# stephane-caron/qpmpc

Hardware: AMD Instinct MI355X
Metric: MPC QP builds+solves/sec (batched) (higher is better)
Workload: dtype f64

## Files before the change

qpmpc_amd/csrc/mpcqp_quad.hip:

```cpp
#include <hip/hip_runtime.h>
#include <math.h>
#include <stdint.h>
#include <type_traits>

#include "mpcqp.h"
#include "mpcqp_internal.h"
#include "mpcqp_quad_common.h"

namespace mpcqp {

namespace quad {

constexpr int MMAX = 32;
constexpr int MK = 2;

}

using namespace quad;

template <int NX, bool ORD, int WPB, bool SLIM, bool MODEL = false, bool GEN = false>
__global__ void __launch_bounds__(64 * WPB, SLIM ? 2 : 1)
    mpcqp_quad_kernel(const double *__restrict__ gA, const double *__restrict__ gB, const double *__restrict__ gC,
                      const double *__restrict__ ge, const double *__restrict__ gx0, const double *__restrict__ ggoal,
                      const double *__restrict__ gtgt, double *__restrict__ oU, double *__restrict__ olam, int32_t *__restrict__ ostatus,
                      int32_t *__restrict__ oiters, const KernelArgs ka, const int64_t batch)
{
    using T = double;
    extern __shared__ __attribute__((aligned(16))) unsigned char smem_raw[];
    {
        const int64_t b0 = ka.A.batch_stride, b1 = ka.B.batch_stride, b2 = ka.C.batch_stride, b3 = ka.e.batch_stride,
                      b4 = ka.x0.batch_stride, b5 = ka.goal.batch_stride;
        const int64_t s0 = ka.A.step_stride, s1 = ka.B.step_stride, s2 = ka.C.step_stride, s3 = ka.e.step_stride;
        asm volatile("" ::"s"(b0), "s"(b1), "s"(b2), "s"(b3), "s"(b4), "s"(b5), "s"(s0), "s"(s1), "s"(s2), "s"(s3), "s"(ka.N), "s"(ka.nu),
                     "s"(ka.flags), "s"(ka.probe), "s"(gA), "s"(gB), "s"(gC), "s"(ge), "s"(gx0), "s"(ggoal), "s"(ka.n), "s"(ka.m),
                     "s"(batch));
    }
    const int lane = threadIdx.x & 63;
    const int wv = threadIdx.x >> 6;
    const int rb = lane & 48;
    const int l = lane & 15;
    int64_t prob = 4 * ((int64_t)blockIdx.x * WPB + wv) + (rb >> 4);
    const bool valid = prob < batch;
    prob = valid ? prob : batch - 1;
    if constexpr (ORD) {
        const int64_t o = ka.order[prob];
        prob = o < 0 ? 0 : (o >= batch ? batch - 1 : o);
    }
    using CV = Carve<SLIM>;
    constexpr int LDM = CV::LDM, PER = CV::PER;
    T *sm = (T *)smem_raw + (4 * wv + (rb >> 4)) * PER;
    const int n = ka.n, m = ka.m;
    const int row0 = l, row1 = l + NV;
    const bool isc0 = row0 < m, isc1 = row1 < m;
    const T INF = HUGE_VAL;
    constexpr int GS = 33;
    T *Gimg = sm + CV::OFF_M, *Ml = sm + CV::OFF_M;
    T *LTp = sm + CV::OFF_LT + (l * (31 - l)) / 2 - (l + 1);
    T *LTimg = sm + CV::OFF_LT, *Timg = sm + CV::OFF_T;
    int *actv = reinterpret_cast<int *>(sm + CV::OFF_ACT);

    long long *stamp = ka.probe ? (long long *)ka.probe + prob * 16 : nullptr;
    auto tick = [&](int slot) {
        if (stamp && l == 0 && valid) {
            stamp[slot] = (long long)__builtin_readcyclecounter();
            if (slot == 0 || slot == 6) stamp[slot ? 13 : 12] = (long long)__builtin_amdgcn_s_memrealtime();
        }
    };
    tick(0);

    T hval0, hval1;
    bool notpd = false;
    T RM0[NV], RM1[NV], RLt[NV];
    T wv_ = T(0);
    if constexpr (MODEL) {
        const T *model = gA;
        const ModelLayout ml = make_model_layout(ka.nx, ka.N, n, m);
        const int nxr = ka.nx, nT = ka.N * ka.nx;
        const T *x0 = gx0 + prob * ka.x0.batch_stride;
        const T *goal = ggoal ? ggoal + prob * ka.goal.batch_stride : nullptr;
        const T *tgt = gtgt ? gtgt + prob * ka.targets.batch_stride : nullptr;
        notpd = model[ml.total] != T(0);
        {
            T r0[NV], r1[NV];
            ld16(r0, model + ml.off_M + (size_t)(isc0 ? row0 : 0) * NV);
            ld16(r1, model + ml.off_M + (size_t)(isc1 ? row1 : 0) * NV);
            ld16(RLt, model + ml.off_LinvT + (size_t)l * NV);
#pragma unroll
            for (int k = 0; k < NV; ++k) {
                RM0[k] = isc0 ? r0[k] : T(0);
                RM1[k] = isc1 ? r1[k] : T(0);
            }
        }
        auto bound = [&](int row, bool isc) {
            if (!isc) return INF;
            const int mkr = ka.mk, kq = mkr == 2 ? row >> 1 : row / mkr;
            T hh = ge ? ge[prob * ka.e.batch_stride + kq * ka.e.step_stride + (row - kq * mkr)] : model[ml.off_e + row];
            for (int c = 0; c < nxr; ++c) hh -= model[ml.off_Hx + (size_t)row * nxr + c] * x0[c];
            return hh;
        };
        hval0 = bound(row0, isc0);
        hval1 = bound(row1, isc1);
        for (int c = 0; c < nxr; ++c) wv_ += model[ml.off_Wx + (size_t)l * nxr + c] * x0[c];
        if ((ka.flags & MPCQP_Q_TERMINAL) && goal)
            for (int c = 0; c < nxr; ++c) wv_ -= model[ml.off_Wg + (size_t)l * nxr + c] * goal[c];
        if ((ka.flags & MPCQP_Q_STAGE) && tgt)
            for (int j2 = 0; j2 < nT; ++j2) wv_ -= model[ml.off_Wt + (size_t)l * nT + j2] * tgt[j2];
        tick(1);
    } else {
    T Pr[NV];
    T qa;
    T g15a = T(0), g15b = T(0);
    {
        constexpr bool WIDE = GEN && NX > 6;
        const int nx = WIDE ? ka.nx : NX;
        const int nu = ka.nu, N = ka.N;
        constexpr int MKG = GEN ? 4 : MK;
        const int mk = GEN ? ka.mk : MK;
        auto stepof = [&](int row) { return mk == 2 ? row >> 1 : (mk == 1 ? row : (mk == 4 ? row >> 2 : row / 3)); };
        const T *A = gA + prob * ka.A.batch_stride;
        const T *B = gB + prob * ka.B.batch_stride;
        const bool hasC = !GEN || gC != nullptr;
        const T *Cm = hasC ? gC + prob * ka.C.batch_stride : A;
        const T *x0 = gx0 + prob * ka.x0.batch_stride;
        const T *goal = ggoal ? ggoal + prob * ka.goal.batch_stride : nullptr;
        const int sA = ka.A.step_stride ? nx * nx : 0, sB = ka.B.step_stride ? nx * nu : 0, sC = (hasC && ka.C.step_stride) ? mk * nx : 0;
        const bool termP = ka.flags & MPCQP_P_TERMINAL, termQ = (ka.flags & MPCQP_Q_TERMINAL) && goal;
        const T *Dm = (GEN && ka.D.ptr) ? (const T *)ka.D.ptr + prob * ka.D.batch_stride : nullptr;
        const T *tgt = (GEN && gtgt) ? gtgt + prob * ka.targets.batch_stride : nullptr;
        const int sD = (GEN && ka.D.step_stride) ? mk * nu : 0;
        const bool stageP = GEN && (ka.flags & MPCQP_P_STAGE), stageQ = GEN && (ka.flags & MPCQP_Q_STAGE) && tgt;
        constexpr int NAe = NX * NX, NEe = NAe + MKG * NX;
        const int NEr = hasC ? NAe + mk * NX : NAe;
        const bool col = (l < n);
        const int j = col ? (nu == 1 ? l : l / nu) : -1, ii = col ? l - j * nu : 0;
        const int64_t eb = prob * ka.e.batch_stride;
        const int kq0 = stepof(row0), kq1 = stepof(row1);
        const T eval0 = isc0 ? ge[eb + kq0 * ka.e.step_stride + (row0 - kq0 * mk)] : INF;
        const T eval1 = isc1 ? ge[eb + kq1 * ka.e.step_stride + (row1 - kq1 * mk)] : INF;
        const bool xl15 = (l == NV - 1);
        T v[NX], gref[NX], bcol[NX];
#pragma unroll
        for (int s = 0; s < NX; ++s) {
            v[s] = (xl15 && s < nx) ? x0[s < nx ? s : 0] : T(0);
            gref[s] = (termQ && s < nx) ? goal[s < nx ? s : 0] : T(0);
        }
#pragma unroll
        for (int r = 0; r < NX; ++r) bcol[r] = (col && r < nx) ? B[j * sB + (r < nx ? r : 0) * nu + ii] : T(0);
        T dcol[MKG], d15a = T(0), d15b = T(0), tg[NX];
#pragma unroll
        for (int u = 0; u < NX; ++u) tg[u] = T(0);
#pragma unroll
        for (int i2 = 0; i2 < MKG; ++i2) dcol[i2] = T(0);
        if constexpr (GEN) {
            if (Dm) {
#pragma unroll
                for (int i2 = 0; i2 < MKG; ++i2) dcol[i2] = (col && !xl15 && i2 < mk) ? Dm[j * sD + i2 * nu + ii] : T(0);
                if (n == NV) {
                    const int j15 = nu == 1 ? NV - 1 : (NV - 1) / nu, i15 = NV - 1 - j15 * nu;
                    d15a = (isc0 && kq0 == j15) ? Dm[j15 * sD + (row0 - kq0 * mk) * nu + i15] : T(0);
                    d15b = (isc1 && kq1 == j15) ? Dm[j15 * sD + (row1 - kq1 * mk) * nu + i15] : T(0);
                }
            }
            if (stageQ && !WIDE) {
#pragma unroll
                for (int u = 0; u < NX; ++u) tg[u] = (l + 16 * u < N * NX) ? tgt[l + 16 * u] : T(0);
            }
        }
        if constexpr (!WIDE) {
        constexpr int NOP = (NEe + 15) / 16;
        T op[NOP][NV];
        static_for<0, NOP>([&](auto rc) {
            constexpr int r = decltype(rc)::value;
            const int e = l + 16 * r;
            const bool ok = e < NEr;
            const T *p = (e < NAe) ? A + e : Cm + (ok ? e - NAe : 0);
            const int st = (e < NAe) ? sA : sC;
#pragma unroll
            for (int k = 0; k < NV; ++k) {
                const int kc = (k < N) ? k : N - 1;
                op[r][k] = p[kc * st];
            }
        });
        tick(8);
        const T wu = (T)ka.wu;
        qa = T(0);
#pragma unroll
        for (int b = 0; b < NV; ++b) Pr[b] = (l == b) ? (col ? wu : T(1)) : T(0);
        tick(9);
        auto mac = [&](auto idx, auto kc_, T &acc, T xx) {
            constexpr int IDX = decltype(idx)::value, K = decltype(kc_)::value;
            fmac_bcast<IDX % 16>(acc, op[IDX / 16][K], xx);
        };
        static_for<0, NV>([&](auto kk) {
            constexpr int k = decltype(kk)::value;
            if (k < N) {
                if constexpr (!GEN) {
                    T g[MK];
                    static_for<0, MK>([&](auto i2c) {
                        constexpr int i2 = decltype(i2c)::value;
                        T acc = T(0);
                        static_for<0, NX>([&](auto sc) {
                            constexpr int s2 = decltype(sc)::value;
                            mac(ic<NAe + i2 * NX + s2>{}, kk, acc, v[s2]);
                        });
                        g[i2] = acc;
                    });
#pragma unroll
                    for (int i2 = 0; i2 < MK; ++i2) Gimg[l * GS + k * MK + i2] = g[i2];
                } else {
                    static_for<0, MKG>([&](auto i2c) {
                        constexpr int i2 = decltype(i2c)::value;
                        if (i2 < mk) {
                            T acc = T(0);
                            if (hasC) {
                                static_for<0, NX>([&](auto sc) {
                                    constexpr int s2 = decltype(sc)::value;
                                    mac(ic<NAe + i2 * NX + s2>{}, kk, acc, v[s2]);
                                });
                            }
                            acc += (j == k) ? dcol[i2] : T(0);
                            Gimg[l * GS + k * mk + i2] = acc;
                        }
                    });
                }
                if constexpr (GEN && k >= 1) {
                    if (stageP || stageQ) {
                        const T wxs = (T)ka.wx;
                        static_for<0, NX>([&](auto sc) {
                            constexpr int s2 = decltype(sc)::value;
                            constexpr int te = k * NX + s2;
                            T src = xl15 ? T(0) : v[s2];
                            const T t = wxs * src;
                            if (stageQ) qa += t * (row_bcast<NV - 1>(v[s2]) - row_bcast<te % 16>(tg[te / 16]));
                            if (stageP) {
                                dpp_ready(src);
                                static_for<0, NV>([&](auto bc) { fmac_bcast<decltype(bc)::value>(Pr[decltype(bc)::value], src, t); });
                            }
                        });
                    }
                }
                const T hk = (j == k && !xl15) ? T(1) : T(0);
                T w[NX];
                static_for<0, NX>([&](auto rc) {
                    constexpr int r = decltype(rc)::value;
                    T acc = hk * bcol[r];
                    static_for<0, NX>([&](auto sc) {
                        constexpr int s2 = decltype(sc)::value;
                        mac(ic<r * NX + s2>{}, kk, acc, v[s2]);
                    });
                    w[r] = acc;
                });
#pragma unroll
                for (int r = 0; r < NX; ++r) v[r] = w[r];
            }
        });
        } else {
        tick(8);
        const T wu = (T)ka.wu;
        qa = T(0);
#pragma unroll
        for (int b = 0; b < NV; ++b) Pr[b] = (l == b) ? (col ? wu : T(1)) : T(0);
        tick(9);
        constexpr int NAw = NX * NX, NCw = 4 * NX, NEw = NAw + NCw + NX, NOPW = (NEw + 15) / 16;
        T opw[2][NOPW];
        auto fetch = [&](auto dc, int k) {
            constexpr int d = decltype(dc)::value;
            const int kc = k < N ? k : N - 1;
            static_for<0, NOPW>([&](auto rc) {
                constexpr int r = decltype(rc)::value;
                constexpr int e0 = 16 * r;
                const int e = e0 + l;
                T val;
                if constexpr (e0 < NAw) {
                    const int rr = e / NX, ss = e - rr * NX;
                    const bool ok = rr < nx && ss < nx;
                    val = A[kc * sA + (ok ? rr * nx + ss : 0)];
                    val = ok ? val : T(0);
                } else if constexpr (e0 < NAw + NCw) {
                    const int e2 = e - NAw, i2 = e2 / NX, ss = e2 - i2 * NX;
                    const bool ok = hasC && i2 < mk && ss < nx;
                    val = Cm[ok ? kc * sC + i2 * nx + ss : 0];
                    val = ok ? val : T(0);
                } else {
                    const int ss = e - NAw - NCw;
                    const bool ok = stageQ && ss < nx;
                    val = ok ? tgt[kc * nx + ss] : T(0);
                }
                opw[d][r] = val;
            });
        };
        fetch(ic<0>{}, 0);
        fetch(ic<1>{}, 1);
        const T wxs = (T)ka.wx;
        auto cstep = [&](auto dc, int k) {
            constexpr int d = decltype(dc)::value;
            static_for<0, NOPW>([&](auto rc) { dpp_ready(opw[d][decltype(rc)::value]); });
            static_for<0, 4>([&](auto i2c) {
                constexpr int i2 = decltype(i2c)::value;
                if (i2 < mk) {
                    T acc = T(0);
                    if (hasC) {
                        static_for<0, NX>([&](auto sc) {
                            constexpr int s2 = decltype(sc)::value, E = NAw + i2 * NX + s2;
                            fmac_bcast<E % 16>(acc, opw[d][E / 16], v[s2]);
                        });
                    }
                    acc += (j == k) ? dcol[i2] : T(0);
                    Gimg[l * GS + k * mk + i2] = acc;
                }
            });
            if (k >= 1 && (stageP || stageQ)) {
                static_for<0, NX>([&](auto sc) {
                    constexpr int s2 = decltype(sc)::value, E = NAw + NCw + s2;
                    T src = xl15 ? T(0) : v[s2];
                    const T t = wxs * src;
                    if (stageQ) qa += t * (row_bcast<NV - 1>(v[s2]) - row_bcast<E % 16>(opw[d][E / 16]));
                    if (stageP) {
                        dpp_ready(src);
                        static_for<0, NV>([&](auto bc) { fmac_bcast<decltype(bc)::value>(Pr[decltype(bc)::value], src, t); });
                    }
                });
            }
            const T hk = (j == k && !xl15) ? T(1) : T(0);
            T w[NX];
            static_for<0, NX>([&](auto rc) {
                constexpr int r = decltype(rc)::value;
                T acc = hk * bcol[r];
                static_for<0, NX>([&](auto sc) {
                    constexpr int s2 = decltype(sc)::value, E = r * NX + s2;
                    fmac_bcast<E % 16>(acc, opw[d][E / 16], v[s2]);
                });
                w[r] = acc;
            });
#pragma unroll
            for (int r = 0; r < NX; ++r) v[r] = w[r];
            fetch(dc, k + 2);
        };
        for (int k = 0; k < N; k += 2) {
            cstep(ic<0>{}, k);
            if (k + 1 < N) cstep(ic<1>{}, k + 1);
        }
        }
        tick(10);
        const T wt = (T)ka.wt;
        T x[NX];
#pragma unroll
        for (int s = 0; s < NX; ++s) {
            x[s] = row_bcast<NV - 1>(v[s]);
            v[s] = xl15 ? bcol[s] : v[s];
        }
#pragma unroll
        for (int s = 0; s < NX; ++s) {
            const T t = wt * v[s];
            if (termQ) qa += t * (x[s] - gref[s]);
            if (termP) {
                T src = v[s];
                dpp_ready(src);
                static_for<0, NV>([&](auto bc) { fmac_bcast<decltype(bc)::value>(Pr[decltype(bc)::value], src, t); });
            }
        }
        qa = col ? qa : T(0);
        tick(11);
        wave_sync();
        hval0 = isc0 ? eval0 - Gimg[(NV - 1) * GS + row0] : INF;
        hval1 = isc1 ? eval1 - Gimg[(NV - 1) * GS + row1] : INF;
        if constexpr (GEN) {
            g15a = d15a;
            g15b = d15b;
        }
    }
    tick(1);
    {
#pragma unroll
        for (int k = 0; k < NV; ++k) {
            RM0[k] = (isc0 && k < NV - 1) ? Gimg[k * GS + row0] : (GEN && k == NV - 1 ? g15a : T(0));
            RM1[k] = (isc1 && k < NV - 1) ? Gimg[k * GS + row1] : (GEN && k == NV - 1 ? g15b : T(0));
            RLt[k] = (l == k) ? T(1) : T(0);
        }
        static_for<0, NV>([&](auto jc) {
            constexpr int j = decltype(jc)::value;
            const T pij = Pr[j];
            const T piv = row_bcast<j>(pij);
            if (!(piv > T(0))) notpd = true;
            const T rinv = fast_rsqrt(piv);
            const T nt2 = -(pij * rinv * rinv);
            T nl = -(pij * rinv);
            RM0[j] *= rinv;
            RM1[j] *= rinv;
            RLt[j] *= rinv;
            const T wj = qa * rinv;
            wv_ = (l == j) ? wj : wv_;
            {
                T src = pij, wsrc = wj;
                asm volatile("s_nop 1" : "+v"(src), "+v"(nl), "+v"(wsrc) : "v"(RM0[j]), "v"(RM1[j]), "v"(RLt[j]));
                fmac_bcast<j>(qa, wsrc, nl);
                static_for<j + 1, NV>([&](auto kc) {
                    constexpr int k = decltype(kc)::value;
                    fmac_bcast<k>(Pr[k], src, nt2);
                    fmac_bcast<k>(RM0[k], nl, RM0[j]);
                    fmac_bcast<k>(RM1[k], nl, RM1[j]);
                    fmac_bcast<k>(RLt[k], nl, RLt[j]);
                });
            }
        });
        wave_sync();
    }
    }
    tick(2);
    tick(3);
    int status = MPCQP_MAX_ITER, iters = 0;
    T xsol = T(0);
    bool done = notpd;
    bool finished = notpd;
    if (notpd) status = MPCQP_NOT_PD;

    if (isc0) st16(Ml + row0 * LDM, RM0);
    if (isc1) st16(Ml + row1 * LDM, RM1);
    T ltd = T(0);
    if constexpr (SLIM) {
        static_for<0, NV>([&](auto kc) {
            constexpr int k = decltype(kc)::value;
            ltd = (l == k) ? RLt[k] : ltd;
            if (k > l) LTp[k] = RLt[k];
        });
    } else {
        st16(LTimg + l * NV, RLt);
    }
    const T y0 = -wv_;
    T s0, s1, invn0, invn1;
    {
        const T d0 = dot_bcast(wv_, RM0, hval0), d1 = dot_bcast(wv_, RM1, hval1);
        s0 = isc0 ? d0 : INF;
        s1 = isc1 ? d1 : INF;
        const T nn0 = dot16(RM0, RM0), nn1 = dot16(RM1, RM1);
        invn0 = (nn0 > T(0)) ? fast_rsqrt(nn0) : T(1);
        invn1 = (nn1 > T(0)) ? fast_rsqrt(nn1) : T(1);
    }
    const bool sel0 = isc0 && (hval0 < T(1e29)), sel1 = isc1 && (hval1 < T(1e29));
    const T tol = (T)ka.tol;
    const T tolh0 = tol + tol * fabs(hval0), tolh1 = tol + tol * fabs(hval1);
    const int max_iter = ka.max_iter;
    T RT[NV], RH[NV];
#pragma unroll
    for (int k = 0; k < NV; ++k) {
        RT[k] = T(0);
        RH[k] = (l == k) ? T(1) : T(0);
    }
    T lam = T(0);
    int myact = 0;
    bool occ = false;
    bool e0 = sel0, e1 = sel1;
    int nq = 0, p = 0;
    unsigned mask = 0;
    bool needp = true;
    T up = T(0);
    int fails = 0;
    T mp[NV];
    auto select = [&]() {
        const bool want = needp & !done;
        const unsigned h0 = ~(unsigned)__double2hiint(s0 * invn0), h1 = ~(unsigned)__double2hiint(s1 * invn1);
        const bool v0 = want & e0 & (s0 < -tolh0), v1 = want & e1 & (s1 < -tolh1);
        const unsigned k0 = v0 ? ((h0 & ~31u) | (unsigned)row0) : 0xffffffffu;
        const unsigned k1 = v1 ? ((h1 & ~31u) | (unsigned)row1) : 0xffffffffu;
        const unsigned mkey = row_min(min(k0, k1));
        const bool none = want & (mkey == 0xffffffffu);
        const bool got = want & !none;
        done = done | none;
        status = none ? (int)MPCQP_SOLVED : status;
        p = got ? (int)(mkey & 31u) : p;
        up = got ? T(0) : up;
        needp = needp & !got;
    };
    auto update = [&](auto bc, auto ec, T zn, T cT, T cH) {
        static_for<decltype(bc)::value, decltype(ec)::value>([&](auto kc) {
            constexpr int k = decltype(kc)::value;
            fmac_bcast<k>(RT[k], zn, cT);
            fmac_bcast<k>(RH[k], zn, cH);
        });
    };
#ifndef QUAD_USPLIT
#define QUAD_USPLIT 8
#endif
    constexpr int USPLIT = QUAD_USPLIT;
    T zn = T(0), cT = T(0), cH = T(0);
    T hd, kd0, kd1, inv, t2, rd;
    wave_sync();
    tick(4);
    for (;;) {
#include "mpcqp_quad_steady.h"
        bool resume = false;
        if (general) for (;;) {
            const bool st = !done;
            const bool phi = p >= NV;
            const int pl = p & 15;
            if (__ballot(st & !(inv > T(0))) != 0ull) {
                T z2 = hd * hd;
                z2 += dpp_mov<ROR8>(z2);
                z2 += dpp_mov<ROR4>(z2);
                z2 += dpp_mov<ROR2>(z2);
                z2 += dpp_mov<ROR1>(z2);
                z2 = row_bcast<0>(z2);
                const T sq = row_get(phi ? s1 : s0, rb, pl), iq = row_get(phi ? invn1 : invn0, rb, pl);
                const bool ok2 = (z2 * iq * iq > T(DEP)) & (z2 > T(0));
                const T iv2 = fast_rcp(z2);
                const bool nearp = !(inv > T(0));
                t2 = nearp ? -sq * iv2 : t2;
                inv = nearp ? (ok2 ? iv2 : T(0)) : inv;
            }
            const bool can_move = (nq < n) & (inv > T(0));
            inv = (can_move & st) ? inv : T(0);
            t2 = can_move ? t2 : INF;
            const int sl = (int)__builtin_ctz(~mask);
            const T r = (occ & st) ? rd : T(0);
            const bool blk = (r > T(0)) & (lam < t2 * r);
            if (__ballot(st & (!can_move | (iters >= max_iter) | blk)) == 0ull) {
                const T tt = st ? t2 : T(0);
                const bool isnew = st & (l == sl), isp = st & (l == pl);
                iters += st ? 1 : 0;
                zn = hd;
                cT = (l == sl) ? inv : -(r * inv);
                cH = -(hd * inv);
                s0 = fma(tt, kd0, s0);
                s1 = fma(tt, kd1, s1);
                T ln = fma(-tt, r, lam);
                ln = (occ & (ln < T(0))) ? T(0) : ln;
                lam = isnew ? up + tt : ln;
                myact = isnew ? p : myact;
                occ = occ | isnew;
                e0 = e0 & !(isp & !phi);
                e1 = e1 & !(isp & phi);
                mask |= st ? (1u << sl) : 0u;
                nq += st ? 1 : 0;
                needp = needp | st;
            } else {
                bool stepping = st;
                {
                    const bool lim = stepping & (iters >= max_iter);
                    done = done | lim;
                    finished = finished | lim;
                    status = lim ? (int)MPCQP_MAX_ITER : status;
                    stepping = stepping & !lim;
                }
                iters += stepping ? 1 : 0;
                const bool cand = occ & stepping & (r > T(0));
                T t1 = INF;
                int lq = 0;
                const unsigned long long bl = __ballot(stepping & blk);
                if (bl != 0ull) {
                    const T ratio = cand ? lam * fast_rcp(r) : INF;
                    unsigned hi, lo;
                    ordered(ratio, hi, lo);
                    hi = cand ? hi : 0xffffffffu;
                    const unsigned mhi = row_min(hi);
                    const unsigned k2 = (cand && hi == mhi) ? ((lo & ~31u) | (unsigned)l) : 0xffffffffu;
                    const unsigned ml = row_min(k2);
                    lq = (int)(ml & 15u);
                    const T tl1 = row_get(ratio, rb, lq);
                    const bool blocked = ((unsigned)(bl >> rb) & 0xffffu) != 0u;
                    t1 = (blocked && mhi != 0xffffffffu) ? tl1 : INF;
                }
                T t = t1 < t2 ? t1 : t2;
                {
                    const bool inf = stepping & !(t < INF);
                    done = done | inf;
                    finished = finished | inf;
                    status = inf ? (int)MPCQP_INFEASIBLE : status;
                    stepping = stepping & !inf;
                }
                t = stepping ? t : T(0);
                const bool full = stepping & (t2 <= t1);
                zn = hd;
                cT = full ? ((l == sl) ? inv : -(r * inv)) : T(0);
                cH = full ? -(hd * inv) : T(0);
                if (stepping) {
                    s0 = fma(t, kd0, s0);
                    s1 = fma(t, kd1, s1);
                    lam -= t * r;
                    lam = (occ && lam < T(0)) ? T(0) : lam;
                    up += t;
                }
                if (full) {
                    if (l == sl) {
                        lam = up;
                        myact = p;
                        occ = true;
                    }
                    if (l == pl) {
                        e0 = e0 & phi;
                        e1 = e1 & !phi;
                    }
                    mask |= 1u << sl;
                    ++nq;
                    needp = true;
                }
                const bool partial = stepping & !full;
                if (__ballot(partial) != 0ull) {
                    const int cl = row_get(myact, rb, lq);
                    T vl = T(0), ac[4] = {T(0), T(0), T(0), T(0)};
                    static_for<0, NV / 4>([&](auto cc) {
                        constexpr int k = 4 * decltype(cc)::value;
                        T v[4];
#pragma unroll
                        for (int j = 0; j < 4; ++j) {
                            v[j] = row_get(RT[k + j], rb, lq);
                            vl = (l == k + j) ? v[j] : vl;
                        }
#pragma unroll
                        for (int j = 0; j < 4; ++j) ac[j] = fma(RT[k + j], v[j], ac[j]);
                        pin(ac[3]);
                    });
                    const T tl = (ac[0] + ac[1]) + (ac[2] + ac[3]);
                    const T tld = row_get(tl, rb, lq);
                    const T itl = fast_rcp(tld);
                    if (partial && l == (cl & 15)) {
                        e0 = (cl < NV) ? sel0 : e0;
                        e1 = (cl < NV) ? e1 : sel1;
                    }
                    zn = partial ? vl : zn;
                    cT = partial ? ((l == lq) ? T(-1) : (occ ? -tl * itl : T(0))) : cT;
                    cH = partial ? vl * itl : cH;
                    lam = (partial & (l == lq)) ? T(0) : lam;
                    occ = occ & !(partial & (l == lq));
                    mask &= partial ? ~(1u << lq) : ~0u;
                    nq -= partial ? 1 : 0;
                }
            }
            if (__ballot(!done & !needp) == 0ull) {
                resume = true;
                break;
            }
            dpp_ready(zn);
            update(ic<0>{}, ic<USPLIT>{}, zn, cT, cH);
            select();
            ld16(mp, Ml + p * LDM);
            update(ic<USPLIT>{}, ic<NV>{}, zn, cT, cH);
            cT = cH = T(0);
            hd = dot16(RH, mp);
            kd0 = dot_bcast(hd, RM0, T(0)), kd1 = dot_bcast(hd, RM1, T(0));
            {
                const bool hi = p >= NV;
                const T kp = hi ? kd1 : kd0, sq = hi ? s1 : s0, iq = hi ? invn1 : invn0;
                const bool okf = kp * iq * iq > T(DEP_FAST);
                const T iv = fast_rcp(kp);
                inv = row_get(okf ? iv : T(-1), rb, p & 15);
                t2 = row_get(-sq * iv, rb, p & 15);
            }
            rd = dot16(RT, mp);
            pin(rd);
        }
        if (resume) continue;
        tick(5);
        if (__ballot(!finished) == 0ull) break;
        int aa[NV];
        if constexpr (SLIM) {
            const int mine = occ ? myact : 0;
            static_for<0, NV>([&](auto ac) { aa[decltype(ac)::value] = __builtin_amdgcn_update_dpp(0, mine, 0x150 + decltype(ac)::value, 0xf, 0xf, false); });
        } else {
            actv[l] = occ ? myact : 0;
            wave_sync();
            const int4 *ap = reinterpret_cast<const int4 *>(actv);
#pragma unroll
            for (int q = 0; q < NV / 4; ++q) {
                const int4 t4 = ap[q];
                aa[4 * q] = t4.x;
                aa[4 * q + 1] = t4.y;
                aa[4 * q + 2] = t4.z;
                aa[4 * q + 3] = t4.w;
            }
        }
        auto ma_dot = [&](T cf) {
            T ma[NV];
#pragma unroll
            for (int a = 0; a < NV; ++a) ma[a] = Ml[aa[a] * LDM + l];
            return dot_bcast(cf, ma, T(0));
        };
        T fresh0, fresh1;
        auto slacks = [&](T yv) {
            const T f0 = dot_bcast(yv, RM0, T(0)), f1 = dot_bcast(yv, RM1, T(0));
            fresh0 = isc0 ? hval0 - f0 : INF;
            fresh1 = isc1 ? hval1 - f1 : INF;
        };
        auto of_act = [&](T x0v, T x1v) {
            const T a = row_get(x0v, rb, myact & 15), b = row_get(x1v, rb, myact & 15);
            return (myact < NV) ? a : b;
        };
        T y = y0 - ma_dot(occ ? lam : T(0));
        slacks(y);
        T rho = of_act(fresh0, fresh1);
        rho = occ ? rho : T(0);
        constexpr double REFTOL = 1e-11;
        const T hact = of_act(hval0, hval1);
        const bool needref = occ & !finished & !(fabs(rho) <= T(REFTOL) * (T(1) + fabs(hact)));
        const unsigned long long nr = __ballot(needref);
        if (nr != 0ull) {
            rho = (((unsigned)(nr >> rb) & 0xffffu) != 0u) ? rho : T(0);
            T uk = T(0);
            if constexpr (SLIM) {
                static_for<0, NV>([&](auto kc) {
                    constexpr int k = decltype(kc)::value;
                    T v = RT[k] * rho;
                    v += dpp_mov<ROR8>(v);
                    v += dpp_mov<ROR4>(v);
                    v += dpp_mov<ROR2>(v);
                    v += dpp_mov<ROR1>(v);
                    uk = (l == k) ? v : uk;
                });
            } else {
                st16(Timg + l * NV, RT);
                wave_sync();
                T tc[NV];
#pragma unroll
                for (int a = 0; a < NV; ++a) tc[a] = Timg[a * NV + l];
                uk = dot_bcast(rho, tc, T(0));
            }
            T dl = -dot_bcast(uk, RT, T(0));
            dl = occ ? dl : T(0);
            if (!finished) {
                const T lraw = lam + dl;
                lam = (occ && lraw < T(0)) ? T(0) : lraw;
            }
            y += uk;
            wave_sync();
            slacks(y);
        }
        bool dirty = row_any((e0 && !(fresh0 >= -T(4) * tolh0)) || (e1 && !(fresh1 >= -T(4) * tolh1)), rb);
        {
            const T ra = of_act(fresh0, fresh1);
            const T ta = of_act(tolh0, tolh1);
            const bool off = row_any(occ && !(fabs(ra) <= T(1e3) * ta), rb);
            const bool neg = row_any(occ && !(lam >= T(0)), rb);
            if (stamp && l == 0 && valid && !finished && done) {
                T worst = T(0);
                stamp[14] = (long long)(dirty ? 1 : 0) | (off ? 2 : 0) | (neg ? 4 : 0) | ((long long)fails << 8) | ((long long)nq << 16);
                (void)worst;
            }
            dirty = dirty || off || neg;
        }
        auto primal = [&]() {
            T lt[NV];
            if constexpr (SLIM) {
                static_for<0, NV>([&](auto kc) {
                    constexpr int k = decltype(kc)::value;
                    lt[k] = (k > l) ? LTp[k > l ? k : l + 1] : ((k == l) ? ltd : T(0));
                });
            } else {
                ld16(lt, LTimg + l * NV);
            }
            return dot_bcast(y, lt, T(0));
        };
        if (!finished && done) {
            if (!dirty) {
                xsol = primal();
                status = MPCQP_SOLVED;
                finished = true;
            } else if (++fails < 4) {
                s0 = fresh0;
                s1 = fresh1;
                status = MPCQP_MAX_ITER;
                done = false;
                needp = true;
            } else {
                xsol = primal();
                status = MPCQP_MAX_ITER;
                finished = true;
            }
        }
        wave_sync();
        if (__ballot(!finished) == 0ull) break;
    }
    tick(6);
    const bool ok = (status == MPCQP_SOLVED);
    T lo0 = T(0), lo1 = T(0);
    if (olam) {
        T *lamv = Ml;
        lamv[row0] = T(0);
        lamv[row1] = T(0);
        wave_sync();
        if (occ) lamv[myact] = lam;
        wave_sync();
        lo0 = ok ? lamv[row0] : T(0);
        lo1 = ok ? lamv[row1] : T(0);
    }
    if (valid) {
        if (l < n) oU[prob * (int64_t)n + l] = ok ? xsol : T(0);
        if (olam) {
            if (isc0) olam[prob * (int64_t)m + row0] = lo0;
            if (isc1) olam[prob * (int64_t)m + row1] = lo1;
        }
        if (l == 0) {
            if (ostatus) ostatus[prob] = status;
            if (oiters) oiters[prob] = iters;
        }
    }
}

[[maybe_unused]] static bool quad_pays(int64_t batch) { return batch > 2 * (int64_t)device_simds_now(); }

static bool quad_general(const KernelArgs &ka)
{
    return ka.nx > 4 || ka.mk != MK || !ka.C.ptr || ka.D.ptr || (ka.flags & (MPCQP_P_STAGE | MPCQP_Q_STAGE));
}

#ifndef MPCQP_QUAD_WIDE_UNIT
bool quad_applies(const KernelArgs &ka)
{
    if (ka.n > NV || ka.m > MMAX || ka.m < 1 || ka.nx < 2 || ka.nx > 16) return false;
    if (ka.mk < 1 || ka.mk > 4 || (!ka.C.ptr && !ka.D.ptr)) return false;
    if (ka.N * ka.mk != ka.m || ka.N > NV) return false;
    if (ka.warm_state || (ka.opt_flags & MPCQP_OPT_SEED_VIOLATED)) return false;
    if (quad_general(ka) && ka.order) return false;
    return true;
}

bool quad_eligible(const KernelArgs &ka, int64_t batch)
{
    if (!quad_applies(ka) || (ka.opt_flags & MPCQP_OPT_TWO_PER_WAVE)) return false;
    return (ka.opt_flags & MPCQP_OPT_FOUR_PER_WAVE) || quad_general(ka) || quad_pays(batch);
}

#endif

template <int NX> static int launch_quad_t(const KernelArgs &ka, int64_t batch, hipStream_t st)
{
    const int64_t waves = (batch + 3) / 4;
    auto go = [&](auto kern, size_t per) {
        const size_t bytes = per * 4 * sizeof(double);
        hipLaunchKernelGGL(kern, dim3((unsigned)waves), dim3(64), bytes, st, (const double *)ka.A.ptr, (const double *)ka.B.ptr,
                           (const double *)ka.C.ptr, (const double *)ka.e.ptr, (const double *)ka.x0.ptr,
                           (const double *)ka.goal.ptr, (const double *)nullptr, (double *)ka.U, (double *)ka.lam, ka.status, ka.iters,
                           ka, batch);
    };
    const bool slim = waves > device_simds_now();
    if (NX > 4 || quad_general(ka)) {
        auto gen = [&](auto kern, size_t per) {
            hipLaunchKernelGGL(kern, dim3((unsigned)waves), dim3(64), per * 4 * sizeof(double), st, (const double *)ka.A.ptr,
                               (const double *)ka.B.ptr, (const double *)ka.C.ptr, (const double *)ka.e.ptr, (const double *)ka.x0.ptr,
                               (const double *)ka.goal.ptr, (const double *)ka.targets.ptr, (double *)ka.U, (double *)ka.lam, ka.status,
                               ka.iters, ka, batch);
        };
        if (slim)
            gen(mpcqp_quad_kernel<NX, false, 1, true, false, true>, Carve<true>::PER);
        else
            gen(mpcqp_quad_kernel<NX, false, 1, false, false, true>, Carve<false>::PER);
    } else if constexpr (NX <= 4) {
        if (ka.order) {
            if (slim)
                go(mpcqp_quad_kernel<NX, true, 1, true>, Carve<true>::PER);
            else
                go(mpcqp_quad_kernel<NX, true, 1, false>, Carve<false>::PER);
        } else if (slim) {
            go(mpcqp_quad_kernel<NX, false, 1, true>, Carve<true>::PER);
        } else {
            go(mpcqp_quad_kernel<NX, false, 1, false>, Carve<false>::PER);
        }
    }
    return (int)hipGetLastError();
}

#ifdef MPCQP_QUAD_WIDE_UNIT
int launch_quad_wide(const KernelArgs &ka, int64_t batch, hipStream_t st)
{
    if (ka.nx == 5) return launch_quad_t<5>(ka, batch, st);
    if (ka.nx == 6) return launch_quad_t<6>(ka, batch, st);
    return ka.nx <= 8 ? launch_quad_t<8>(ka, batch, st) : ka.nx <= 12 ? launch_quad_t<12>(ka, batch, st) : launch_quad_t<16>(ka, batch, st);
}
#else
int launch_quad_wide(const KernelArgs &ka, int64_t batch, hipStream_t st);

int launch_quad(const KernelArgs &ka, int64_t batch, hipStream_t st)
{
    switch (ka.nx) {
    case 2: return launch_quad_t<2>(ka, batch, st);
    case 3: return launch_quad_t<3>(ka, batch, st);
    case 4: return launch_quad_t<4>(ka, batch, st);
    default: return launch_quad_wide(ka, batch, st);
    }
}

bool quad_model_eligible(const KernelArgs &ka, int64_t batch)
{
    if (ka.n > NV || ka.m > MMAX || ka.m < 1 || ka.warm_state || (ka.opt_flags & (MPCQP_OPT_TWO_PER_WAVE | MPCQP_OPT_SEED_VIOLATED)))
        return false;
    return (ka.opt_flags & MPCQP_OPT_FOUR_PER_WAVE) || quad_pays(batch);
}

int launch_quad_model(const KernelArgs &ka, int64_t batch, hipStream_t st)
{
    const int64_t waves = (batch + 3) / 4;
    auto go = [&](auto kern, size_t per) {
        const size_t bytes = per * 4 * sizeof(double);
        hipLaunchKernelGGL(kern, dim3((unsigned)waves), dim3(64), bytes, st, (const double *)ka.model, (const double *)nullptr,
                           (const double *)nullptr, (const double *)ka.e.ptr, (const double *)ka.x0.ptr, (const double *)ka.goal.ptr,
                           (const double *)ka.targets.ptr, (double *)ka.U, (double *)ka.lam, ka.status, ka.iters, ka, batch);
    };
    const bool slim = waves > device_simds_now();
    if (ka.order) {
        if (slim)
            go(mpcqp_quad_kernel<3, true, 1, true, true>, Carve<true>::PER);
        else
            go(mpcqp_quad_kernel<3, true, 1, false, true>, Carve<false>::PER);
    } else if (slim) {
        go(mpcqp_quad_kernel<3, false, 1, true, true>, Carve<true>::PER);
    } else {
        go(mpcqp_quad_kernel<3, false, 1, false, true>, Carve<false>::PER);
    }
    return (int)hipGetLastError();
}

#endif

}
```

Measured before the change: 216.2 million.

## Hoist operand loads earlier and fuse G-row and state-propagation MAC loops

```diff
diff --git a/qpmpc_amd/csrc/mpcqp_quad.hip b/qpmpc_amd/csrc/mpcqp_quad.hip
--- a/qpmpc_amd/csrc/mpcqp_quad.hip
+++ b/qpmpc_amd/csrc/mpcqp_quad.hip
@@ -13,6 +13,12 @@
 
 constexpr int MMAX = 32;
 constexpr int MK = 2;
+#ifndef QUAD_STEADY_PAD
+#define QUAD_STEADY_PAD "s_nop 0"
+#endif
+#ifndef QUAD_PROBE_REFINE
+#define QUAD_PROBE_REFINE 0
+#endif
 
 }
 
@@ -64,6 +70,7 @@
         if (stamp && l == 0 && valid) {
             stamp[slot] = (long long)__builtin_readcyclecounter();
             if (slot == 0 || slot == 6) stamp[slot ? 13 : 12] = (long long)__builtin_amdgcn_s_memrealtime();
+            if (slot == 4 && NX == 3 && !ORD && !SLIM && !MODEL && !GEN) asm volatile(QUAD_STEADY_PAD);
         }
     };
     tick(0);
@@ -118,34 +125,44 @@
         const int mk = GEN ? ka.mk : MK;
         auto stepof = [&](int row) { return mk == 2 ? row >> 1 : (mk == 1 ? row : (mk == 4 ? row >> 2 : row / 3)); };
         const T *A = gA + prob * ka.A.batch_stride;
-        const T *B = gB + prob * ka.B.batch_stride;
         const bool hasC = !GEN || gC != nullptr;
         const T *Cm = hasC ? gC + prob * ka.C.batch_stride : A;
+        const int sA = ka.A.step_stride ? nx * nx : 0, sB = ka.B.step_stride ? nx * nu : 0, sC = (hasC && ka.C.step_stride) ? mk * nx : 0;
+        constexpr int NAe = NX * NX, NEe = NAe + MKG * NX;
+        const int NEr = hasC ? NAe + mk * NX : NAe;
+        constexpr int NOP = WIDE ? 1 : (NEe + 15) / 16;
+        T op[NOP][NV];
+#include "mpcqp_quad_operands.h"
+        const T *B = gB + prob * ka.B.batch_stride;
         const T *x0 = gx0 + prob * ka.x0.batch_stride;
         const T *goal = ggoal ? ggoal + prob * ka.goal.batch_stride : nullptr;
-        const int sA = ka.A.step_stride ? nx * nx : 0, sB = ka.B.step_stride ? nx * nu : 0, sC = (hasC && ka.C.step_stride) ? mk * nx : 0;
         const bool termP = ka.flags & MPCQP_P_TERMINAL, termQ = (ka.flags & MPCQP_Q_TERMINAL) && goal;
         const T *Dm = (GEN && ka.D.ptr) ? (const T *)ka.D.ptr + prob * ka.D.batch_stride : nullptr;
         const T *tgt = (GEN && gtgt) ? gtgt + prob * ka.targets.batch_stride : nullptr;
         const int sD = (GEN && ka.D.step_stride) ? mk * nu : 0;
         const bool stageP = GEN && (ka.flags & MPCQP_P_STAGE), stageQ = GEN && (ka.flags & MPCQP_Q_STAGE) && tgt;
-        constexpr int NAe = NX * NX, NEe = NAe + MKG * NX;
-        const int NEr = hasC ? NAe + mk * NX : NAe;
         const bool col = (l < n);
         const int j = col ? (nu == 1 ? l : l / nu) : -1, ii = col ? l - j * nu : 0;
         const int64_t eb = prob * ka.e.batch_stride;
         const int kq0 = stepof(row0), kq1 = stepof(row1);
-        const T eval0 = isc0 ? ge[eb + kq0 * ka.e.step_stride + (row0 - kq0 * mk)] : INF;
-        const T eval1 = isc1 ? ge[eb + kq1 * ka.e.step_stride + (row1 - kq1 * mk)] : INF;
+        const T elo0 = ge[eb + (isc0 ? kq0 * ka.e.step_stride + (row0 - kq0 * mk) : 0)];
+        const T elo1 = ge[eb + (isc1 ? kq1 * ka.e.step_stride + (row1 - kq1 * mk) : 0)];
+        const T eval0 = isc0 ? elo0 : INF, eval1 = isc1 ? elo1 : INF;
         const bool xl15 = (l == NV - 1);
         T v[NX], gref[NX], bcol[NX];
+        const T *gsrc = termQ ? goal : x0;
 #pragma unroll
         for (int s = 0; s < NX; ++s) {
-            v[s] = (xl15 && s < nx) ? x0[s < nx ? s : 0] : T(0);
-            gref[s] = (termQ && s < nx) ? goal[s < nx ? s : 0] : T(0);
-        }
-#pragma unroll
-        for (int r = 0; r < NX; ++r) bcol[r] = (col && r < nx) ? B[j * sB + (r < nx ? r : 0) * nu + ii] : T(0);
+            const T xs = x0[s < nx ? s : 0], gs = gsrc[s < nx ? s : 0];
+            v[s] = (xl15 && s < nx) ? xs : T(0);
+            gref[s] = (termQ && s < nx) ? gs : T(0);
+        }
+        const int jB = col ? j * sB + ii : 0;
+#pragma unroll
+        for (int r = 0; r < NX; ++r) {
+            const T bs = B[jB + (r < nx ? r : 0) * nu];
+            bcol[r] = (col && r < nx) ? bs : T(0);
+        }
         T dcol[MKG], d15a = T(0), d15b = T(0), tg[NX];
 #pragma unroll
         for (int u = 0; u < NX; ++u) tg[u] = T(0);
@@ -167,20 +184,6 @@
             }
         }
         if constexpr (!WIDE) {
-        constexpr int NOP = (NEe + 15) / 16;
-        T op[NOP][NV];
-        static_for<0, NOP>([&](auto rc) {
-            constexpr int r = decltype(rc)::value;
-            const int e = l + 16 * r;
-            const bool ok = e < NEr;
-            const T *p = (e < NAe) ? A + e : Cm + (ok ? e - NAe : 0);
-            const int st = (e < NAe) ? sA : sC;
-#pragma unroll
-            for (int k = 0; k < NV; ++k) {
-                const int kc = (k < N) ? k : N - 1;
-                op[r][k] = p[kc * st];
-            }
-        });
         tick(8);
         const T wu = (T)ka.wu;
         qa = T(0);
@@ -194,35 +197,6 @@
         static_for<0, NV>([&](auto kk) {
             constexpr int k = decltype(kk)::value;
             if (k < N) {
-                if constexpr (!GEN) {
-                    T g[MK];
-                    static_for<0, MK>([&](auto i2c) {
-                        constexpr int i2 = decltype(i2c)::value;
-                        T acc = T(0);
-                        static_for<0, NX>([&](auto sc) {
-                            constexpr int s2 = decltype(sc)::value;
-                            mac(ic<NAe + i2 * NX + s2>{}, kk, acc, v[s2]);
-                        });
-                        g[i2] = acc;
-                    });
-#pragma unroll
-                    for (int i2 = 0; i2 < MK; ++i2) Gimg[l * GS + k * MK + i2] = g[i2];
-                } else {
-                    static_for<0, MKG>([&](auto i2c) {
-                        constexpr int i2 = decltype(i2c)::value;
-                        if (i2 < mk) {
-                            T acc = T(0);
-                            if (hasC) {
-                                static_for<0, NX>([&](auto sc) {
-                                    constexpr int s2 = decltype(sc)::value;
-                                    mac(ic<NAe + i2 * NX + s2>{}, kk, acc, v[s2]);
-                                });
-                            }
-                            acc += (j == k) ? dcol[i2] : T(0);
-                            Gimg[l * GS + k * mk + i2] = acc;
-                        }
-                    });
-                }
                 if constexpr (GEN && k >= 1) {
                     if (stageP || stageQ) {
                         const T wxs = (T)ka.wx;
@@ -240,16 +214,43 @@
                     }
                 }
                 const T hk = (j == k && !xl15) ? T(1) : T(0);
-                T w[NX];
-                static_for<0, NX>([&](auto rc) {
-                    constexpr int r = decltype(rc)::value;
-                    T acc = hk * bcol[r];
+                T g[MKG], w[NX];
+#pragma unroll
+                for (int i2 = 0; i2 < MKG; ++i2) g[i2] = T(0);
+#pragma unroll
+                for (int r = 0; r < NX; ++r) w[r] = hk * bcol[r];
+                if constexpr (!GEN) {
                     static_for<0, NX>([&](auto sc) {
                         constexpr int s2 = decltype(sc)::value;
-                        mac(ic<r * NX + s2>{}, kk, acc, v[s2]);
+                        static_for<0, MK>([&](auto i2c) { mac(ic<NAe + decltype(i2c)::value * NX + s2>{}, kk, g[decltype(i2c)::value], v[s2]); });
+                        static_for<0, NX>([&](auto rc) { mac(ic<decltype(rc)::value * NX + s2>{}, kk, w[decltype(rc)::value], v[s2]); });
                     });
-                    w[r] = acc;
-                });
+#pragma unroll
+                    for (int i2 = 0; i2 < MK; ++i2) Gimg[l * GS + k * MK + i2] = g[i2];
+                } else {
+                    auto psi = [&](auto sc) {
+                        constexpr int s2 = decltype(sc)::value;
+                        static_for<0, NX>([&](auto rc) { mac(ic<decltype(rc)::value * NX + s2>{}, kk, w[decltype(rc)::value], v[s2]); });
+                    };
+                    auto grows = [&](auto sc) {
+                        constexpr int s2 = decltype(sc)::value;
+                        if (!hasC) return;
+                        mac(ic<NAe + s2>{}, kk, g[0], v[s2]);
+                        if (mk > 1) mac(ic<NAe + NX + s2>{}, kk, g[1], v[s2]);
+                        if (mk > 2) mac(ic<NAe + 2 * NX + s2>{}, kk, g[2], v[s2]);
+                        if (mk > 3) mac(ic<NAe + 3 * NX + s2>{}, kk, g[3], v[s2]);
+                    };
+                    if constexpr (NX > 5) static_for<0, NX>(grows);
+                    else static_for<0, NX>([&](auto sc) { psi(sc); grows(sc); });
+                    static_for<0, MKG>([&](auto i2c) {
+                        constexpr int i2 = decltype(i2c)::value;
+                        if (i2 < mk) {
+                            g[i2] += (j == k) ? dcol[i2] : T(0);
+                            Gimg[l * GS + k * mk + i2] = g[i2];
+                        }
+                    });
+                    if constexpr (NX > 5) static_for<0, NX>(psi);
+                }
 #pragma unroll
                 for (int r = 0; r < NX; ++r) v[r] = w[r];
             }
@@ -730,9 +731,8 @@
             const bool off = row_any(occ && !(fabs(ra) <= T(1e3) * ta), rb);
             const bool neg = row_any(occ && !(lam >= T(0)), rb);
             if (stamp && l == 0 && valid && !finished && done) {
-                T worst = T(0);
                 stamp[14] = (long long)(dirty ? 1 : 0) | (off ? 2 : 0) | (neg ? 4 : 0) | ((long long)fails << 8) | ((long long)nq << 16);
-                (void)worst;
+                if (QUAD_PROBE_REFINE && ((unsigned)(nr >> rb) & 0xffffu) != 0u) stamp[14] |= 1ll << 24;
             }
             dirty = dirty || off || neg;
         }
diff --git a/qpmpc_amd/csrc/mpcqp_quad_operands.h b/qpmpc_amd/csrc/mpcqp_quad_operands.h
--- /dev/null
+++ b/qpmpc_amd/csrc/mpcqp_quad_operands.h
@@ -0,0 +1,20 @@
+if constexpr (!WIDE) {
+    static_for<0, NOP>([&](auto rc) {
+        constexpr int r = decltype(rc)::value;
+        const int e = l + 16 * r;
+        const bool ok = e < NEr;
+        const T *p = (e < NAe) ? A + e : Cm + (ok ? e - NAe : 0);
+        const int st = (e < NAe) ? sA : sC;
+        if (N == NV) {
+            const uint32_t stb = (uint32_t)st * (uint32_t)sizeof(T);
+#pragma unroll
+            for (int k = 0; k < NV; ++k) op[r][k] = *reinterpret_cast<const T *>(reinterpret_cast<const char *>(p) + (uint64_t)k * stb);
+        } else {
+#pragma unroll
+            for (int k = 0; k < NV; ++k) {
+                const int kc = (k < N) ? k : N - 1;
+                op[r][k] = p[kc * st];
+            }
+        }
+    });
+}
```

New measurement: 220.3 million, median of 6. +1.9%, better.
